# ssheybani/baby-vision-curriculum

Hardware: AMD Instinct MI355X
Metric: video clips/sec (node) VideoMAE-base 16x224^2 bf16 pretraining (higher is better)
Workload: dtype bf16; 1 GPU; VideoMAE-base (ViT-B/16 encoder, 4-layer decoder), 16x224x224 clips, tubelet 2, 90% tube mask, full training step (fwd + MSE + bwd + GradScaler + SGD-Nesterov); clips_per_gpu=256, global_batch=256, parallelism=dp1, weights=random init N(0,0.02), seed 0

## Files before the change

baby-vision-curriculum_amd/csrc/attention.hip:

```cpp
#include <stdlib.h>

#include "attention.h"

namespace bvc {

#define AS3 __attribute__((address_space(3)))
#define MFMA32(a, b, c) __builtin_amdgcn_mfma_f32_32x32x16_bf16((a), (b), (c), 0, 0, 0)

template <int HD>
__device__ __forceinline__ int swz_dual(int r) {
    if constexpr (HD == 64) return (((r >> 1) & 1) << 2) | ((r >> 2) & 3);
    else return (r >> 2) & 3;
}

template <int HD>
constexpr int pan_w(int p) { return HD - 64 * p >= 64 ? 64 : HD - 64 * p; }
constexpr int img_hd(int hd) { return hd == 80 || hd == 88 ? 96 : hd; }
constexpr uint32_t kDmaZero = 0xfffffff0u;
__device__ __forceinline__ int swz_pw(int pw, int r) { return pw == 64 ? swz_dual<64>(r) : swz_dual<32>(r); }

template <int PW, int NW, int VC = PW / 8>
__device__ __forceinline__ void stage_panel(__amdgpu_buffer_rsrc_t rs, int row0, int ld, int col0, char* lds, int GB, int wave, int lane) {
    constexpr int CPR = PW / 8;
    constexpr int RPP = 64 / CPR;
// ... 10 lines not shown
    }
}

template <int HD, int NW = 4, int HV = HD>
__device__ __forceinline__ void stage64(__amdgpu_buffer_rsrc_t rs, int row0, int ld, int col0, char* lds,
                                        int wave, int lane) {
    static_assert(HV == HD || (HD == 96 && HV > 64 && HV % 8 == 0), "stage64: a narrower head only on the 96 image");
    if constexpr (HD > 64) {
        stage_panel<64, NW>(rs, row0, ld, col0, lds, 16 * HD * 2, wave, lane);
        stage_panel<pan_w<HD>(1), NW, (HV - 64) / 8>(rs, row0, ld, col0 + 64, lds + 2048, 16 * HD * 2, wave, lane);
        return;
    }
    constexpr int CPR = HD / 8;
    constexpr int RPP = 64 / CPR;
#pragma unroll
    for (int jj = 0; jj < (HD / 8 + NW - 1) / NW; ++jj) {
        const int j = wave + NW * jj;
        if (NW > HD / 8 && j >= HD / 8) break;
        const int r = RPP * j + lane / CPR;
        const int c = (lane % CPR) ^ swz_dual<HD>(r);
        const uint32_t off = (uint32_t)(((size_t)(row0 + r) * ld + col0 + c * 8) * 2);
        glds16(rs, off, __builtin_amdgcn_readfirstlane((uint32_t)(size_t)((AS3 char*)lds) + (uint32_t)j * 1024u));
    }
}

template <int HD>
struct FragAddr {
    uint32_t rows[HD / 16];
    uint32_t tr[HD / 32][2];
};

template <int HD>
__device__ __forceinline__ FragAddr<HD> make_frag_addr(int lane) {
    FragAddr<HD> a;
    if constexpr (HD > 64) {
        constexpr int GB = 16 * HD * 2;
        const int r = lane & 31, h = lane >> 5, rg = r & 15;
#pragma unroll
        for (int st = 0; st < HD / 16; ++st) {
            const int pw = pan_w<HD>(st >> 2);
            a.rows[st] = (r >> 4) * GB + (st >> 2) * 2048 + rg * pw * 2 + (((2 * (st & 3) + h) ^ swz_pw(pw, rg)) << 4);
        }
        const int q = (lane >> 2) & 3, p = lane & 3;
#pragma unroll
        for (int t = 0; t < HD / 32; ++t) {
            const int pw = pan_w<HD>(t >> 1);
// ... 554 lines not shown
        bf16_t* krow = dqkv + (size_t)(b * N + ki) * ld + D + head * HD;
        bf16_t* vrow = krow + D;
#pragma unroll
        for (int t = 0; t < HI / 32; ++t)
#pragma unroll
            for (int g = 0; g < 4; ++g) {
                const int d = 32 * t + 8 * g + 4 * h;
                if (HD != HI && d >= HD) continue;
                uint2 a = {pack2bf(dk[t][4 * g] * scale, dk[t][4 * g + 1] * scale), pack2bf(dk[t][4 * g + 2] * scale, dk[t][4 * g + 3] * scale)};
                *reinterpret_cast<uint2*>(krow + d) = a;
                uint2 e = {pack2bf(dv[t][4 * g], dv[t][4 * g + 1]), pack2bf(dv[t][4 * g + 2], dv[t][4 * g + 3])};
                *reinterpret_cast<uint2*>(vrow + d) = e;
            }
    }
}

template <int HD, int NBT>
__global__ __launch_bounds__(320, 1) void attn_bwd_head_kernel(const bf16_t* __restrict__ qkv, const bf16_t* __restrict__ dctx,
                                                               const bf16_t* __restrict__ ctx, const float* __restrict__ lse,
                                                               bf16_t* __restrict__ dqkv, int N, int H, int D, int nheads,
                                                               uint32_t qkv_bytes, uint32_t dctx_bytes, float scale, float scale_log2) {
    static_assert(HD == 64, "whole-head backward: head_dim 64");
    extern __shared__ __attribute__((aligned(16))) char smem[];
    constexpr int IMG = 192 * HD * 2, SUB = 32 * HD * 2, KS = 16 * HD * 2;
    constexpr int QI = 0, KI = IMG, VI = 2 * IMG, OI = 3 * IMG;
    constexpr int STAT = 4 * IMG;
    constexpr int DST = STAT + 2 * 192 * 4;
    const AS3 char* lds = (const AS3 char*)smem;
    const int tid = threadIdx.x, lane = tid & 63;
    const int wave = __builtin_amdgcn_readfirstlane(tid >> 6);
    const int ld = 3 * D, h = lane >> 5;
    const int NB = NBT > 0 ? NBT : (N + 31) >> 5;
    const __amdgpu_buffer_rsrc_t rq = make_rsrc(qkv, qkv_bytes), rd = make_rsrc(dctx, dctx_bytes);
    const FragAddr<HD> fa = make_frag_addr<HD>(lane);
    const FragAddr<32> fs = make_frag_addr<32>(lane);

    auto stage_qvo = [&](int bh) __attribute__((always_inline)) {
        if (wave < 4) {
            const int b = bh / H, head = bh % H, row0 = b * N;
            for (int rb = 0; rb * 64 < N; ++rb) {
                stage64<HD>(rq, row0 + rb * 64, ld, head * HD, smem + QI + rb * 2 * SUB, wave, lane);
                stage64<HD>(rq, row0 + rb * 64, ld, 2 * D + head * HD, smem + VI + rb * 2 * SUB, wave, lane);
                stage64<HD>(rd, row0 + rb * 64, D, head * HD, smem + OI + rb * 2 * SUB, wave, lane);
            }
        }
    };
    auto stage_k = [&](int bh) __attribute__((always_inline)) {
        if (wave < 4) {
            const int b = bh / H, head = bh % H, row0 = b * N;
            for (int rb = 0; rb * 64 < N; ++rb) stage64<HD>(rq, row0 + rb * 64, ld, D + head * HD, smem + KI + rb * 2 * SUB, wave, lane);
        }
    };
    float st_lse = 0.f, st_del[5];
    auto load_stats = [&](int bh) __attribute__((always_inline)) {
        const int b = bh / H, head = bh % H;
        st_lse = (tid < N) ? lse[(size_t)bh * N + tid] : 0.f;
#pragma unroll
        for (int k = 0; k < 5; ++k) {
            const int q = (tid >> 3) + 40 * k, c = tid & 7;
            float acc = 0.f;
            if (q < N) {
                const bf16x8 dv = load8(dctx + (size_t)(b * N + q) * D + head * HD + 8 * c);
                const bf16x8 ov = load8(ctx + (size_t)(b * N + q) * D + head * HD + 8 * c);
#pragma unroll
                for (int j = 0; j < 8; ++j) acc += bf2f((bf16_t)dv[j]) * bf2f((bf16_t)ov[j]);
            }
            st_del[k] = acc;
        }
    };
    auto store_stats = [&]() __attribute__((always_inline)) {
        AS3 float* st = (AS3 float*)((AS3 char*)smem + STAT);
        if (tid < 192) st[tid] = st_lse;
#pragma unroll
        for (int k = 0; k < 5; ++k) {
            float acc = st_del[k];
            acc += __shfl_xor(acc, 1, 64);
            acc += __shfl_xor(acc, 2, 64);
            acc += __shfl_xor(acc, 4, 64);
            const int q = (tid >> 3) + 40 * k;
            if ((tid & 7) == 0 && q < 192) st[192 + q] = -acc;
        }
    };

    int bh = blockIdx.x;
    if (bh >= nheads) return;
    load_stats(bh);
    stage_qvo(bh);
    stage_k(bh);
    for (; bh < nheads; bh += gridDim.x) {
    const int b = bh / H, head = bh % H;
    const int nxt = bh + gridDim.x;
    asm volatile("s_waitcnt vmcnt(0)" ::: "memory");
    store_stats();
    __syncthreads();

    for (int kb = wave; kb < NB; kb += 5) {
        const int ki = kb * 32 + (lane & 31);
        bf16x8 kf[HD / 16], vf[HD / 16];
#pragma unroll
        for (int st = 0; st < HD / 16; ++st) {
            kf[st] = *reinterpret_cast<const AS3 bf16x8*>(lds + KI + kb * SUB + fa.rows[st]);
            vf[st] = *reinterpret_cast<const AS3 bf16x8*>(lds + VI + kb * SUB + fa.rows[st]);
        }
        f32x16 dk[HD / 32], dv[HD / 32];
#pragma unroll
        for (int t = 0; t < HD / 32; ++t) { dk[t] = zero16(); dv[t] = zero16(); }
        const bool key_ok = ki < N;
#pragma unroll
        for (int qb = 0; qb < (NBT > 0 ? NBT : NB); ++qb) {
            const AS3 char* qim = lds + QI + qb * SUB;
            const AS3 char* oim = lds + OI + qb * SUB;
            const AS3 float* stl = reinterpret_cast<const AS3 float*>(lds + STAT) + qb * 32 + 4 * h;
            f32x16 s = zero16(), dp;
#pragma unroll
            for (int g = 0; g < 4; ++g) {
                const f32x4 nd = *reinterpret_cast<const AS3 f32x4*>(stl + 192 + 8 * g);
#pragma unroll
                for (int e = 0; e < 4; ++e) dp[4 * g + e] = nd[e];
            }
#pragma unroll
            for (int stp = 0; stp < HD / 16; ++stp) {
                s = MFMA32(*reinterpret_cast<const AS3 bf16x8*>(qim + fa.rows[stp]), kf[stp], s);
                dp = MFMA32(*reinterpret_cast<const AS3 bf16x8*>(oim + fa.rows[stp]), vf[stp], dp);
            }
// ... 46 lines not shown
#pragma unroll
                for (int g = 0; g < 4; ++g) {
                    const int d = 32 * t + 8 * g + 4 * h;
                    uint2 a = {pack2bf(dk[t][4 * g] * scale, dk[t][4 * g + 1] * scale), pack2bf(dk[t][4 * g + 2] * scale, dk[t][4 * g + 3] * scale)};
                    *reinterpret_cast<uint2*>(krow + d) = a;
                    uint2 e = {pack2bf(dv[t][4 * g], dv[t][4 * g + 1]), pack2bf(dv[t][4 * g + 2], dv[t][4 * g + 3])};
                    *reinterpret_cast<uint2*>(vrow + d) = e;
                }
        }
    }
    __syncthreads();
    if (nxt < nheads) {
        stage_qvo(nxt);
        load_stats(nxt);
    }

    for (int qb = wave; qb < NB; qb += 5) {
        const int qi = qb * 32 + (lane & 31);
        f32x16 dq[HD / 32];
#pragma unroll
        for (int t = 0; t < HD / 32; ++t) dq[t] = zero16();
#pragma unroll
        for (int kb = 0; kb < (NBT > 0 ? NBT : NB); ++kb) {
            const AS3 char* kim = lds + KI + kb * SUB;
            const AS3 char* blk = lds + DST + (kb * 5 + qb) * 2048;
            const bf16x8 b0 = lds_tr<0>(blk, fs.tr[0][0], fs.tr[0][1]);
            const bf16x8 b1 = lds_tr<1024>(blk, fs.tr[0][0], fs.tr[0][1]);
#pragma unroll
            for (int t = 0; t < HD / 32; ++t) dq[t] = MFMA32(lds_tr<0>(kim, fa.tr[t][0], fa.tr[t][1]), b0, dq[t]);
#pragma unroll
            for (int t = 0; t < HD / 32; ++t) dq[t] = MFMA32(lds_tr<KS>(kim, fa.tr[t][0], fa.tr[t][1]), b1, dq[t]);
        }
        if (qi < N) {
            bf16_t* orow = dqkv + (size_t)(b * N + qi) * ld + head * HD;
#pragma unroll
            for (int t = 0; t < HD / 32; ++t)
#pragma unroll
                for (int g = 0; g < 4; ++g) {
                    const int d = 32 * t + 8 * g + 4 * h;
                    uint2 a = {pack2bf(dq[t][4 * g] * scale, dq[t][4 * g + 1] * scale), pack2bf(dq[t][4 * g + 2] * scale, dq[t][4 * g + 3] * scale)};
                    *reinterpret_cast<uint2*>(orow + d) = a;
                }
        }
    }
    __syncthreads();
    if (nxt < nheads) stage_k(nxt);
    }
}

static int xcd_remap() {
#ifdef BVC_EXPERIMENTS
    return getenv("BVC_ATTN_PLAIN_GRID") == nullptr;
#else
    return 1;
#endif
}

static bool head_kernel_enabled() {
#ifdef BVC_EXPERIMENTS
    return getenv("BVC_ATTN_NO_HEAD_KERNEL") == nullptr;
#else
    return true;
#endif
}

template <int HD>
static int fwd_hd(const bf16_t* qkv, bf16_t* ctx, float* lse, int B, int N, int H, hipStream_t stream, float sm_scale) {
    constexpr int HI = img_hd(HD);
    const int D = H * HD;
// ... 7 lines not shown
        BVC_CHECK_HIP(hipGetLastError());
        return BVC_OK;
    }
#endif
    const dim3 grid((unsigned)(((N + 127) / 128) * B * H));
    hipLaunchKernelGGL((attn_fwd_kernel<HD, 4>), grid, dim3(256), 4 * 64 * HI * 2, stream, qkv, ctx, lse, N, H, D, (uint32_t)bytes, scale_log2,
                       xcd_remap());
    BVC_CHECK_HIP(hipGetLastError());
    return BVC_OK;
}

template <int HD>
static int bwd_hd(const bf16_t* qkv, const bf16_t* ctx, const bf16_t* dctx, const float* lse, float* delta, bf16_t* dqkv, int B,
                  int N, int H, hipStream_t stream, float sm_scale, int parts) {
    constexpr int HI = img_hd(HD);
    const int D = H * HD;
    const size_t bytes = (size_t)B * N * 3 * D * 2;
    const float scale = sm_scale > 0.f ? sm_scale : 1.0f / sqrtf((float)HD), scale_log2 = scale * 1.4426950408889634f;
    const dim3 grid((unsigned)(((N + 127) / 128) * B * H));
    const int remap = xcd_remap();
    if constexpr (HD == 64) {
        if (parts == 3 && N <= 160 && head_kernel_enabled()) {
            constexpr size_t lds = 4 * 192 * HD * 2 + 2 * 192 * 4 + 25 * 2048;
            static bool attr_set = false;
            if (!attr_set) {
                BVC_CHECK_HIP(hipFuncSetAttribute(reinterpret_cast<const void*>(&attn_bwd_head_kernel<HD, 5>),
                                                  hipFuncAttributeMaxDynamicSharedMemorySize, (int)lds));
                BVC_CHECK_HIP(hipFuncSetAttribute(reinterpret_cast<const void*>(&attn_bwd_head_kernel<HD, 0>),
                                                  hipFuncAttributeMaxDynamicSharedMemorySize, (int)lds));
                attr_set = true;
            }
            static int ncu = 0;
            if (ncu == 0) {
                int dev = 0;
                hipDeviceProp_t prop;
                BVC_CHECK_HIP(hipGetDevice(&dev));
                BVC_CHECK_HIP(hipGetDeviceProperties(&prop, dev));
                ncu = prop.multiProcessorCount > 0 ? prop.multiProcessorCount : 256;
            }
            const int nheads = B * H;
            const dim3 g((unsigned)(nheads < ncu ? nheads : ncu));
            if (N > 128)
                hipLaunchKernelGGL((attn_bwd_head_kernel<HD, 5>), g, dim3(320), lds, stream, qkv, dctx, ctx, lse, dqkv, N, H, D, nheads,
                                   (uint32_t)bytes, (uint32_t)((size_t)B * N * D * 2), scale, scale_log2);
            else
                hipLaunchKernelGGL((attn_bwd_head_kernel<HD, 0>), g, dim3(320), lds, stream, qkv, dctx, ctx, lse, dqkv, N, H, D, nheads,
                                   (uint32_t)bytes, (uint32_t)((size_t)B * N * D * 2), scale, scale_log2);
            BVC_CHECK_HIP(hipGetLastError());
            return BVC_OK;
        }
    }
    if (parts & 1) {
#ifdef BVC_EXPERIMENTS
    if (HI == HD && getenv("BVC_ATTN_DQ_W") != nullptr) {
        constexpr int NB = 3;
        const dim3 gridw((unsigned)(((N + 32 * NB - 1) / (32 * NB)) * B * H));
        hipLaunchKernelGGL((attn_bwd_dq_w_kernel<HI, NB>), gridw, dim3(64), kRing * 2 * 32 * HI * 2, stream, qkv, dctx, ctx, lse, delta, dqkv, N, H, D,
                           (uint32_t)bytes, scale, scale_log2, remap);
    } else
#endif
    hipLaunchKernelGGL(attn_bwd_dq_kernel<HD>, grid, dim3(256), 4 * 64 * HI * 2, stream, qkv, dctx, ctx, lse, delta, dqkv, N, H, D,
                       (uint32_t)bytes, scale, scale_log2, remap);
    }
    if (parts & 2) {
    constexpr int lds_dkdv = 2 * (2 * 64 * HI * 2 + 512);
    if constexpr (lds_dkdv > 65536) {
// ... 51 lines not shown
```

baby-vision-curriculum_amd/csrc/rowops.h:

```cpp
#pragma once
#include "common.h"
#include "dropgate.h"

namespace bvc {

struct RowMap { int rin, rout, roff; };
static inline RowMap identity_rows() { return RowMap{0, 0, 0}; }

struct PatchGeom { int T, C, H, W, ts, ps; };

struct PixelSrc {
    const void* ptr;
    int is_u8;
    float mean[4], stdv[4];
};
static inline PixelSrc pixels_f32(const float* p) { return PixelSrc{p, 0, {0, 0, 0, 0}, {1, 1, 1, 1}}; }

int launch_ln_fwd(const float* x, RowMap rm, const float* gamma, const float* beta, bf16_t* y, float* mean, float* rstd,
                  int M, int D, float eps, hipStream_t s, float* y32 = nullptr);
size_t ln_bwd_workspace_floats(int M, int D);
size_t ln_bwd_workspace_floats_upto(int Mmax, int D);
int launch_ln_bwd(const bf16_t* dy, const float* x, RowMap rm, const float* mean, const float* rstd, const float* gamma,
                  float* dres, int accumulate, bf16_t* dres_bf, float* dgamma, float* dbeta, float* part, int M, int D, hipStream_t s,
                  const Gate* gate = nullptr);
int launch_ln_param_reduce(const float* part, int nblk, int D, float* dgamma, float* dbeta, hipStream_t s);
int launch_colsum_bf16(const bf16_t* X, int M, int N, int ld, float alpha, float* out, hipStream_t s);
int launch_colsum_bf16_scaled(const bf16_t* X, int M, int N, int ld, float alpha, const float* alpha_dev, float* out, hipStream_t s);
int launch_colsum_f32(const float* X, RowMap rm, int M, int D, float* out, hipStream_t s);
int launch_token_mean(const float* x, int B, int N, int D, float* out, hipStream_t s);
int launch_token_mean_bwd(const float* dmean, int B, int N, int D, float* dx, hipStream_t s);
int launch_fcnorm_bwd_bcast(const float* dy, const float* p, const float* mean, const float* rstd, const float* gamma, float* dres,
                            bf16_t* dres_bf, float* dgamma, float* dbeta, int B, int N, int D, hipStream_t s, const Gate* gate = nullptr);
int launch_dropout_mask(const Gate& gate, size_t n, uint8_t* out, hipStream_t s);
void dropout_mask_host(const Gate& gate, size_t n, uint8_t* out);
int launch_cast_bf16(const float* in, bf16_t* out, size_t n, hipStream_t s);
int launch_gather_rows_bf16(const float* in, RowMap rm, bf16_t* out, int M, int D, hipStream_t s);
int launch_mask_index(const uint8_t* mask, int B, int L, int nvis, int nmask, int* vis_idx, int* msk_idx, int* status, hipStream_t s);
int launch_dual_mask_index(const uint8_t* mask, const uint8_t* decode, int B, int L, int nvis, int ndec, int* vis_idx, int* dec_idx,
                           int* status, hipStream_t s);
int launch_gather_patches(PixelSrc clip, const int* vis_idx, bf16_t* A, int B, int nvis, PatchGeom pg, hipStream_t s);
int launch_labels(PixelSrc clip, const int* dec_idx, float* labels, int B, int ndec, PatchGeom pg, int norm_pix, hipStream_t s);
int launch_fill_masked(float* xfull, const float* mask_token, const float* pos, const int* dec_idx, int B, int Ld, int nvis,
                       int ndec, int D, hipStream_t s);
int launch_sgd_step(float* p, float* g, float* buf, size_t n, float lr, float momentum, float dampening, float wd, int nesterov,
                    int first, int maximize, const float* grad_scale, const float* found_inf, int write_grad, bf16_t* shadow,
                    hipStream_t s);
int launch_adam_prep(float* state, double lr, double beta1, double beta2, const float* found_inf, hipStream_t s);
int launch_adam_step(float* p, float* g, float* m, float* v, size_t n, double lr, double beta1, double beta2, double eps, double wd,
                     int decoupled, int maximize, const float* state, const float* grad_scale, const float* found_inf, int write_grad,
                     bf16_t* shadow, hipStream_t s);
int launch_sgd_step_segments(float* p, float* g, float* buf, int64_t n, const int64_t* seg_start, const int* seg_group, const int* blk_seg,
                             int nseg, const bvc_sgd_groups* groups, const float* grad_scale, const float* found_inf, int write_grad,
                             bf16_t* shadow, hipStream_t s);
int launch_adam_step_segments(float* p, float* g, float* m, float* v, int64_t n, const int64_t* seg_start, const int* seg_group,
                              const int* blk_seg, int nseg, const bvc_adam_groups* groups, float* state, double* hyper_dev,
                              const float* grad_scale, const float* found_inf, int write_grad, bf16_t* shadow, hipStream_t s);
int launch_pad_heads(const bf16_t* wqkv, const float* bqkv, const bf16_t* wo, bf16_t* wqkv_p, float* bqkv_p, bf16_t* wo_p, int D, int H,
                     int hd, int hdp, hipStream_t s);
int launch_unpad_head_grads(const float* gwqkv_p, const float* gbqkv_p, const float* gwo_p, float* gwqkv, float* gbqkv, float* gwo, int D,
// ... 18 lines not shown
```

baby-vision-curriculum_amd/csrc/rowops.hip:

```cpp
#include "rowops.h"
#include "gemm.h"

#include <algorithm>

namespace bvc {

constexpr int kMaxChunks = 4;
constexpr int kWideChunks = 6;

__device__ __forceinline__ int map_row(int m, RowMap rm) {
    return rm.rin > 0 ? (m / rm.rin) * rm.rout + rm.roff + (m % rm.rin) : m;
}

template <int LPR>
__device__ __forceinline__ float row_sum(float v) {
#pragma unroll
    for (int o = LPR / 2; o > 0; o >>= 1) v += __shfl_xor(v, o, 64);
    return v;
}

template <int LPR, int NC>
__global__ __launch_bounds__(256) void ln_fwd_kernel(const float* __restrict__ x, RowMap rm, const float* __restrict__ gamma,
                                                     const float* __restrict__ beta, bf16_t* __restrict__ y, float* __restrict__ y32,
                                                     float* __restrict__ mean, float* __restrict__ rstd, int M, int D, float eps) {
// ... 405 lines not shown
#pragma unroll
    for (int e = 0; e < 4; ++e)
        if (q * 4 + e < n) out[q * 4 + e] = r[e] >= gate.thr ? 1 : 0;
}

__global__ void cast_f32_bf16_kernel(const float* __restrict__ in, bf16_t* __restrict__ out, size_t n) {
    const size_t i = ((size_t)blockIdx.x * blockDim.x + threadIdx.x) * 8;
    if (i + 8 <= n) {
        const f32x4 a = *reinterpret_cast<const f32x4*>(in + i);
        const f32x4 b = *reinterpret_cast<const f32x4*>(in + i + 4);
        *reinterpret_cast<uint4*>(out + i) = uint4{pack2bf(a[0], a[1]), pack2bf(a[2], a[3]), pack2bf(b[0], b[1]), pack2bf(b[2], b[3])};
    } else {
        for (size_t j = i; j < n; ++j) out[j] = f2bf(in[j]);
    }
}

__global__ void gather_rows_bf16_kernel(const float* __restrict__ in, RowMap rm, bf16_t* __restrict__ out, int M, int D) {
    const size_t i = (size_t)blockIdx.x * blockDim.x + threadIdx.x;
    const int nch = D >> 2;
    if (i >= (size_t)M * nch) return;
    const int m = (int)(i / nch), c = (int)(i % nch);
    const f32x4 v = *reinterpret_cast<const f32x4*>(in + (size_t)map_row(m, rm) * D + c * 4);
    *reinterpret_cast<uint2*>(out + (size_t)m * D + c * 4) = uint2{pack2bf(v[0], v[1]), pack2bf(v[2], v[3])};
}

__global__ void mask_index_kernel(const uint8_t* __restrict__ mask, int L, int nvis, int nmask, int* __restrict__ vis_idx,
                                  int* __restrict__ msk_idx, int* __restrict__ status) {
    const int b = blockIdx.x, lane = threadIdx.x;
    int nv = 0, nm = 0;
    const unsigned long long below = lane == 0 ? 0ull : (~0ull >> (64 - lane));
    for (int base = 0; base < L; base += 64) {
        const int t = base + lane;
        const bool in = t < L;
        const bool mk = in && mask[(size_t)b * L + t] != 0;
        const unsigned long long bm = __ballot(mk), bv = __ballot(in && !mk);
        if (mk) { const int p = nm + __popcll(bm & below); if (p < nmask) msk_idx[(size_t)b * nmask + p] = t; }
        if (in && !mk) { const int p = nv + __popcll(bv & below); if (p < nvis) vis_idx[(size_t)b * nvis + p] = t; }
        nm += __popcll(bm);
        nv += __popcll(bv);
    }
    if (lane == 0 && (nv != nvis || nm != nmask)) atomicOr(status, 1);
}

__global__ void dual_mask_index_kernel(const uint8_t* __restrict__ mask, const uint8_t* __restrict__ decode, int L, int nvis, int ndec,
                                       int* __restrict__ vis_idx, int* __restrict__ dec_idx, int* __restrict__ status) {
    const int b = blockIdx.x, lane = threadIdx.x;
// ... 884 lines not shown
            hipLaunchKernelGGL(fcnorm_bwd_bcast_gate_kernel, dim3(std::max(chunks, pcols), B + 1), dim3(256), 0, s, dy, p, mean, rstd, gamma, dres,
                               dres_bf, dgamma, dbeta, B, N, D, B, *gate);
        } else {
            hipLaunchKernelGGL(fcnorm_bwd_bcast_kernel, dim3(std::max(chunks, pcols), B + 1), dim3(256), 0, s, dy, p, mean, rstd, gamma, dres,
                               dres_bf, dgamma, dbeta, B, N, D, B);
        }
    }
    BVC_CHECK_HIP(hipGetLastError());
    return BVC_OK;
}

int launch_cast_bf16(const float* in, bf16_t* out, size_t n, hipStream_t s) {
    hipLaunchKernelGGL(cast_f32_bf16_kernel, dim3(blocks_for((n + 7) / 8)), dim3(256), 0, s, in, out, n);
    BVC_CHECK_HIP(hipGetLastError());
    return BVC_OK;
}

int launch_gather_rows_bf16(const float* in, RowMap rm, bf16_t* out, int M, int D, hipStream_t s) {
    hipLaunchKernelGGL(gather_rows_bf16_kernel, dim3(blocks_for((size_t)M * (D / 4))), dim3(256), 0, s, in, rm, out, M, D);
    BVC_CHECK_HIP(hipGetLastError());
    return BVC_OK;
}

int launch_mask_index(const uint8_t* mask, int B, int L, int nvis, int nmask, int* vis_idx, int* msk_idx, int* status, hipStream_t s) {
    hipLaunchKernelGGL(mask_index_kernel, dim3(B), dim3(64), 0, s, mask, L, nvis, nmask, vis_idx, msk_idx, status);
    BVC_CHECK_HIP(hipGetLastError());
    return BVC_OK;
}

int launch_dual_mask_index(const uint8_t* mask, const uint8_t* decode, int B, int L, int nvis, int ndec, int* vis_idx, int* dec_idx,
                           int* status, hipStream_t s) {
    hipLaunchKernelGGL(dual_mask_index_kernel, dim3(B), dim3(64), 0, s, mask, decode, L, nvis, ndec, vis_idx, dec_idx, status);
    BVC_CHECK_HIP(hipGetLastError());
    return BVC_OK;
}

int launch_gather_patches(PixelSrc clip, const int* vis_idx, bf16_t* A, int B, int nvis, PatchGeom pg, hipStream_t s) {
    BVC_REQUIRE(pg.ps % 8 == 0 && pg.W % 4 == 0, "gather_patches: patch size must be a multiple of 8");
    const size_t items = (size_t)B * nvis * (pg.C * pg.ts * pg.ps * pg.ps / 8);
    hipLaunchKernelGGL(gather_patches_kernel, dim3(blocks_for(items)), dim3(256), 0, s, clip, vis_idx, A, B, nvis, pg);
    BVC_CHECK_HIP(hipGetLastError());
    return BVC_OK;
}

int launch_labels(PixelSrc clip, const int* dec_idx, float* labels, int B, int ndec, PatchGeom pg, int norm_pix, hipStream_t s) {
    BVC_REQUIRE(pg.ps % 4 == 0, "labels: patch size must be a multiple of 4");
// ... 227 lines not shown
```

baby-vision-curriculum_amd/csrc/videomae.hip:

```cpp
#include <math.h>
#include <stdarg.h>
#include <stdio.h>
#include <stdlib.h>
#include <string.h>

#include <algorithm>
#include <string>
#include <vector>

#include "stack.h"

namespace bvc {
static thread_local char g_err[1024] = "";
void set_error(const char* fmt, ...) {
    va_list ap;
    va_start(ap, fmt);
    vsnprintf(g_err, sizeof(g_err), fmt, ap);
    va_end(ap);
}
const char* last_error() { return g_err; }
}

using namespace bvc;

// ... 306 lines not shown
    }
    const RowMap tail{ndec, Ld, nvis};
    TRY(launch_ln_fwd(c->dec.x_out, tail, params + L.norm_w, params + L.norm_b, c->lnf, c->meanf, c->rstdf, Mm, Dd, cf.decoder_norm_eps, st));
    TRY(launch_labels(pixels, c->dec_idx, c->labels, B, ndec, pg, cf.norm_pix_loss, st));
    {
        GemmProblem p = gemm(c->lnf, (size_t)Mm * Dd, Dd, c->wbf + L.head_w, (size_t)P * Dd, Dd, Mm, P, Dd, EPI_LOSS, c->diff, P);
        p.bias = params + L.head_b; p.labels = c->labels; p.partial = c->partial; p.C2 = logits;
        c->npartial = gemm_num_tiles(p, -1);
        TRY(launch_gemm(&p, 1, GEMM_NT, -1, st));
    }
    TRY(launch_loss_finalize(c->partial, c->npartial, (double)Mm * (double)P, c->status, loss, st));
    c->have_forward = true;
    return BVC_OK;
}

int bvc_videomae_backward(bvc_ctx* c, const float* grad_loss, float* G, bvc_bucket_fn on_bucket, void* user, void* stream) {
    BVC_REQUIRE(c && grad_loss && G, "backward: null argument");
    if (!c->have_forward) { set_error("backward: no forward state (call bvc_videomae_forward first; one backward per forward)"); return BVC_ERR_STATE; }
    c->have_forward = false;
    hipStream_t st = (hipStream_t)stream;
    const bvc_videomae_config& cf = c->cfg;
    const Layout& L = c->lay;
    const int B = c->batch, nvis = c->nvis, ndec = c->ndec, Ld = c->Ld;
    const int Mv = B * nvis, Md = B * Ld, Mm = B * ndec;
    const int D = cf.hidden_size, Dd = cf.decoder_hidden_size, P = c->P;
    const bf16_t* W = c->wbf;
    const float* params = c->params;
    auto bucket = [&](int64_t lo, int64_t hi) { if (on_bucket) on_bucket(lo, hi - lo, user); };
    begin_backward(c->w);

    BVC_CHECK_HIP(hipMemsetAsync(G, 0, (size_t)L.total * 4, st));
    const float cmse = (float)(2.0 / ((double)Mm * (double)P));
    {
        GemmProblem p = gemm(c->diff, (size_t)Mm * P, P, c->lnf, (size_t)Mm * Dd, Dd, P, Dd, Mm, EPI_F32, G + L.head_w, Dd);
        p.alpha = cmse; p.alpha_dev = grad_loss;
        p.rowsum = G + L.head_b;
        const int tile = plan_dw(&p, 1);
        TRY(launch_gemm(&p, 1, GEMM_TN, tile, st));
    }
    {
        GemmProblem p = gemm(c->diff, (size_t)Mm * P, P, W + L.head_w, (size_t)P * Dd, Dd, Mm, Dd, P, EPI_BF16, c->w.dln, Dd);
        p.alpha = cmse; p.alpha_dev = grad_loss;
        TRY(launch_gemm(&p, 1, GEMM_NN, -1, st));
    }
    BVC_CHECK_HIP(hipMemsetAsync(c->dres_dec, 0, (size_t)Md * Dd * 4, st));
    BVC_CHECK_HIP(hipMemsetAsync(c->w.dyb[0], 0, (size_t)Md * Dd * 2, st));
    const RowMap tail{ndec, Ld, nvis};
    TRY(launch_ln_bwd(c->w.dln, c->dec.x_out, tail, c->meanf, c->rstdf, params + L.norm_w, c->dres_dec, 0, c->w.dyb[0],
                      G + L.norm_w, G + L.norm_b, c->w.ln_part, Mm, Dd, st));
    bucket(L.norm_w, L.total);
    for (int i = c->dec.nlayers - 1; i >= 0; --i) {
        TRY(layer_backward(c->w, c->dec, i, L.dec[i], c->dec.act[i].x_in, c->dres_dec, G, B, Ld, st, on_bucket, user));
    }
    TRY(launch_colsum_f32(c->dres_dec, tail, Mm, Dd, G + L.mask_token, st));
    const RowMap headrows{nvis, Ld, 0};
    TRY(launch_gather_rows_bf16(c->dres_dec, headrows, c->de2d, Mv, Dd, st));
    {
        GemmProblem p = gemm(c->de2d, (size_t)Mv * Dd, Dd, c->xe_bf, (size_t)Mv * D, D, Dd, D, Mv, EPI_F32, G + L.e2d_w, D);
        const int tile = plan_dw(&p, 1);
        TRY(launch_gemm(&p, 1, GEMM_TN, tile, st));
    }
    {
        GemmProblem p = gemm(c->de2d, (size_t)Mv * Dd, Dd, W + L.e2d_w, (size_t)Dd * D, D, Mv, D, Dd, EPI_F32_BF16, c->dres_enc, D);
        p.C2 = c->w.dyb[c->w.seq % 3];
        TRY(launch_gemm(&p, 1, GEMM_NN, -1, st));
    }
    bucket(L.e2d_w, L.dec.front().ln1w);
    for (int i = c->enc.nlayers - 1; i >= 0; --i) {
        TRY(layer_backward(c->w, c->enc, i, L.enc[i], c->enc.act[i].x_in, c->dres_enc, G, B, nvis, st, on_bucket, user));
    }
    {
        GemmProblem p = gemm(c->w.dyb[c->w.seq % 3], (size_t)Mv * D, D, c->Ape, (size_t)Mv * c->Kp, c->Kp, D, c->Kp, Mv, EPI_F32, G + L.pe_w, c->Kp);
        p.rowsum = G + L.pe_b;
        const int tile = plan_dw(&p, 1);
        TRY(launch_gemm(&p, 1, GEMM_TN, tile, st));
    }
    TRY(join_side(c->w, c->w.seq & 1, st, on_bucket, user));
    TRY(join_side(c->w, (c->w.seq + 1) & 1, st, on_bucket, user));
// ... 554 lines not shown
```

baby-vision-curriculum_amd/jepa.py:

```python
from __future__ import annotations

import ctypes
import math
from functools import partial

import numpy as np
import torch
import torch.nn as nn

from . import _lib
from .dropgate import BranchGate
from .flat import FlatParamModule, query_layout


def apply_masks(x, masks):
    all_x = []
    for m in masks:
        mask_keep = m.unsqueeze(-1).repeat(1, 1, x.size(-1))
        all_x += [torch.gather(x, dim=1, index=mask_keep)]
    return torch.cat(all_x, dim=0)


def repeat_interleave_batch(x, B, repeat):
    N = len(x) // B
# ... 109 lines not shown

    @property
    def num_patches(self):
        return self._pe_info.num_patches

    @property
    def drop_path_scale(self):
        return self._gate.scale

    def _get_ctx(self, batch):
        dev = self._flat.device.index
        if self._ctx is not None and self._ctx_key[1] == dev and self._ctx_key[0] >= batch:
            return self._ctx
        self._free_ctx()
        h = ctypes.c_void_p()
        _lib.check(_lib.lib().bvc_vit_create(ctypes.byref(self._cfg), batch, ctypes.byref(h)), "bvc_vit_create")
        self._ctx, self._ctx_key = h, (batch, dev)
        return h

    def _free_ctx(self):
        if getattr(self, "_ctx", None) is not None:
            _lib.lib().bvc_vit_destroy(self._ctx)
            self._ctx = None

    def __del__(self):
        try:
            self._free_ctx()
        except Exception:
            pass

    def _run_forward(self, imgs, idx):
        B = imgs.shape[0]
        N = idx.shape[1] if idx is not None else self.num_patches
        h = self._get_ctx(B)
        out = torch.empty((B, N, self.embed_dim), dtype=torch.float32, device=imgs.device)
        fmt = _lib.pixel_format(imgs, self.pixel_mean, self.pixel_std, self.in_chans)
        self._shadow_vouch(h)
        if self.training and self._gate.enabled:
            self._gate.arm(_lib.lib().bvc_vit_set_drop, h, imgs.device, B, N)
        _lib.check(_lib.lib().bvc_vit_forward_px(h, imgs.data_ptr(), ctypes.byref(fmt) if fmt is not None else None,
                                                 idx.data_ptr() if idx is not None else None, B, N, self._flat.data_ptr(),
                                                 out.data_ptr(), _lib.current_stream_ptr()), "bvc_vit_forward")
        self._shadow_established(h)
        self._live = (imgs, idx)
        return out

# ... 80 lines not shown
        self._init_flat(layout, numel, init, frozen=("predictor_pos_embed",))
        self._ctx, self._ctx_key = None, None

    @property
    def drop_path_scale(self):
        return self._gate.scale

    def _get_ctx(self, B, nsets, tokens):
        dev = self._flat.device.index
        k = self._ctx_key
        if self._ctx is not None and k[3] == dev and k[0] >= B and k[1] >= nsets and k[2] >= tokens:
            return self._ctx
        self._free_ctx()
        h = ctypes.c_void_p()
        tokens = max(tokens, min(2 * self.num_patches, tokens + 64))
        _lib.check(_lib.lib().bvc_predictor_create(ctypes.byref(self._cfg), B, nsets, tokens, ctypes.byref(h)), "bvc_predictor_create")
        self._ctx, self._ctx_key = h, (B, nsets, tokens, dev)
        return h

    def _free_ctx(self):
        if getattr(self, "_ctx", None) is not None:
            _lib.lib().bvc_predictor_destroy(self._ctx)
            self._ctx = None

    def __del__(self):
        try:
            self._free_ctx()
        except Exception:
            pass

    def _run_forward(self, z, idx_ctx, idx_pred):
        B, Nc = idx_ctx.shape
        nsets, _, Np = idx_pred.shape
        h = self._get_ctx(B, nsets, Nc + Np)
        zf = z.detach().to(torch.float32).contiguous()
        out = torch.empty((nsets * B, Np, self.embed_dim), dtype=torch.float32, device=z.device)
        self._shadow_vouch(h)
        if self.training and self._gate.enabled:
            self._gate.arm(_lib.lib().bvc_predictor_set_drop, h, z.device, nsets * B, Nc + Np)
        _lib.check(_lib.lib().bvc_predictor_forward(h, zf.data_ptr(), idx_ctx.data_ptr(), idx_pred.data_ptr(), B, Nc, nsets, Np,
                                                    self._flat.data_ptr(), out.data_ptr(), _lib.current_stream_ptr()),
                   "bvc_predictor_forward")
        self._shadow_established(h)
        self._live = (zf, idx_ctx, idx_pred)
        return out

# ... 207 lines not shown
```

baby-vision-curriculum_amd/videomae.py:

```python
from __future__ import annotations

import ctypes
import warnings
from dataclasses import dataclass
from typing import Optional

import torch
import torch.nn as nn

from . import _lib
from .dropgate import BranchGate
from .flat import FlatParamModule, query_layout


class VideoMAEConfig:

    def __init__(self, image_size=224, patch_size=16, num_channels=3, num_frames=16, tubelet_size=2,
                 hidden_size=768, num_hidden_layers=12, num_attention_heads=12, intermediate_size=3072,
                 hidden_act="gelu", layer_norm_eps=1e-12, initializer_range=0.02, qkv_bias=True,
                 use_mean_pooling=True, decoder_num_attention_heads=6, decoder_hidden_size=384,
                 decoder_num_hidden_layers=4, decoder_intermediate_size=1536, norm_pix_loss=True,
                 hidden_dropout_prob=0.0, attention_probs_dropout_prob=0.0, drop_path_rate=0.0,
                 output_hidden_states=False, output_attentions=False, **kwargs):
        self.output_hidden_states, self.output_attentions = bool(output_hidden_states), bool(output_attentions)
# ... 139 lines not shown
            "bool_decode_pos: the number of decoded patches per clip changed (or differs between clips, or a decoded patch was not "
            "masked) without a new model object; every clip must decode the same number of its masked patches",
            "every clip must have the same number of decoded patches")
        self.pixel_mean, self.pixel_std = 0.5, 0.25

    def _get_ctx(self, batch, nmask, ndec=None):
        key = (batch, nmask, self._flat.device.index, nmask if ndec is None else ndec)
        if self._ctx is not None and self._ctx_key[1:] == key[1:] and self._ctx_key[0] >= batch:
            return self._ctx
        self._free_ctx()
        h = ctypes.c_void_p()
        cc = self.config.to_c()
        if ndec is None:
            _lib.check(_lib.lib().bvc_videomae_create(ctypes.byref(cc), batch, nmask, ctypes.byref(h)), "bvc_videomae_create")
        else:
            _lib.check(_lib.lib().bvc_videomae_create_dual(ctypes.byref(cc), batch, nmask, ndec, ctypes.byref(h)), "bvc_videomae_create_dual")
        self._ctx, self._ctx_key = h, key
        return h

    def _free_ctx(self):
        if self._ctx is not None:
            _lib.lib().bvc_videomae_destroy(self._ctx)
            self._ctx = None

    def __del__(self):
        try:
            self._free_ctx()
        except Exception:
            pass

    def _num_masked(self, mask):
        return self._mask_count.count(mask, self.strict_mask_check)

    def _num_decoded(self, decode, mask):
        return self._decode_count.count(decode, self.strict_mask_check, bad=(decode & ~mask).any(),
                                        bad_message="bool_decode_pos must be a subset of bool_masked_pos: a decoded patch is visible to the encoder")

    def _run_forward(self, pixels, mask, decode, want_logits):
        cfg = self.config
        fmt = _lib.pixel_format(pixels, self.pixel_mean, self.pixel_std, cfg.num_channels)
        B = pixels.shape[0]
        nmask = self._num_masked(mask)
        ndec = self._num_decoded(decode, mask) if decode is not None else None
        h = self._get_ctx(B, nmask, ndec)
        loss = torch.empty((), dtype=torch.float32, device=pixels.device)
        logits = None
# ... 238 lines not shown
        self._ctx = None
        self._ctx_key = None
        self._train = _TrainCtx()
        self._warned_eval_grad = False
        self.pixel_mean, self.pixel_std = 0.5, 0.25

    def _get_ctx(self, batch):
        key = (batch, self._flat.device.index)
        if self._ctx is not None and self._ctx_key[1] == key[1] and self._ctx_key[0] >= batch:
            return self._ctx
        self._free_ctx()
        h = ctypes.c_void_p()
        cc = self.config.to_c()
        _lib.check(_lib.lib().bvc_videomae_encoder_create(ctypes.byref(cc), batch, ctypes.byref(h)), "bvc_videomae_encoder_create")
        self._ctx, self._ctx_key = h, key
        return h

    def _get_train_ctx(self, batch):
        t = self._train
        key = (batch, self._flat.device.index)
        if t.h is not None and t.key[1] == key[1] and t.key[0] >= batch:
            return t.h
        t.free()
        h = ctypes.c_void_p()
        cc = self.config.to_c()
        _lib.check(_lib.lib().bvc_videomae_cls_create(ctypes.byref(cc), batch, ctypes.byref(h)), "bvc_videomae_cls_create")
        t.h, t.key = h, key
        return h

    def _shadow_ctx(self):
        return self._train.h

    def __deepcopy__(self, memo):
        import copy
        new = super().__deepcopy__(memo)
        new.fc_norm = copy.deepcopy(self.fc_norm, memo)
        new.classifier = copy.deepcopy(self.classifier, memo)
        return new

    def _free_ctx(self):
        if self._ctx is not None:
            _lib.lib().bvc_videomae_encoder_destroy(self._ctx)
            self._ctx = None

    def __del__(self):
        try:
# ... 149 lines not shown
```

Measured before the change: 3281 clips/s.

## Double-buffer K in whole-head attention backward and zero only head rows in decoder grad

For the N=160 whole-head attention backward, the K image is double-buffered in LDS with exact 160-row staging. The next head's K is prefetched right after the stats barrier instead of after a trailing __syncthreads, which removes that barrier and overlaps the load with compute. Separately, the full memsets of the decoder residual gradient buffers are replaced by a kernel that zeroes only the visible head rows, because the tail rows are overwritten by layer-norm backward. The Python destroy paths also invalidate shadow state. The extra LDS image raises LDS use per block, and the narrower zeroing depends on the tail rows really being overwritten.

Result: no change. 3282 clips/s (median of 3 runs) (+0.0%).

```diff
diff --git a/baby-vision-curriculum_amd/csrc/attention.hip b/baby-vision-curriculum_amd/csrc/attention.hip
--- a/baby-vision-curriculum_amd/csrc/attention.hip
+++ b/baby-vision-curriculum_amd/csrc/attention.hip
@@ -56,6 +56,13 @@
         const uint32_t off = (uint32_t)(((size_t)(row0 + r) * ld + col0 + c * 8) * 2);
         glds16(rs, off, __builtin_amdgcn_readfirstlane((uint32_t)(size_t)((AS3 char*)lds) + (uint32_t)j * 1024u));
     }
+}
+
+__device__ __forceinline__ void stage32(__amdgpu_buffer_rsrc_t rs, int row0, int ld, int col0, char* lds, int wave, int lane) {
+    const int r = 8 * wave + lane / 8;
+    const int c = (lane % 8) ^ swz_dual<64>(r);
+    const uint32_t off = (uint32_t)(((size_t)(row0 + r) * ld + col0 + c * 8) * 2);
+    glds16(rs, off, __builtin_amdgcn_readfirstlane((uint32_t)(size_t)((AS3 char*)lds) + (uint32_t)wave * 1024u));
 }
 
 template <int HD>
@@ -656,9 +663,12 @@
                                                                uint32_t qkv_bytes, uint32_t dctx_bytes, float scale, float scale_log2) {
     static_assert(HD == 64, "whole-head backward: head_dim 64");
     extern __shared__ __attribute__((aligned(16))) char smem[];
-    constexpr int IMG = 192 * HD * 2, SUB = 32 * HD * 2, KS = 16 * HD * 2;
+    constexpr bool K2 = NBT == 5;
+    constexpr int ROWS = K2 ? 160 : 192;
+    constexpr int IMG = ROWS * HD * 2, SUB = 32 * HD * 2, KS = 16 * HD * 2;
     constexpr int QI = 0, KI = IMG, VI = 2 * IMG, OI = 3 * IMG;
-    constexpr int STAT = 4 * IMG;
+    constexpr int KJ = 4 * IMG;
+    constexpr int STAT = (K2 ? 5 : 4) * IMG;
     constexpr int DST = STAT + 2 * 192 * 4;
     const AS3 char* lds = (const AS3 char*)smem;
     const int tid = threadIdx.x, lane = tid & 63;
@@ -669,20 +679,35 @@
     const FragAddr<HD> fa = make_frag_addr<HD>(lane);
     const FragAddr<32> fs = make_frag_addr<32>(lane);
 
+    auto stage_img = [&](__amdgpu_buffer_rsrc_t rs, int row0, int ldi, int col0, char* img) __attribute__((always_inline)) {
+        if constexpr (K2) {
+            stage64<HD>(rs, row0, ldi, col0, img, wave, lane);
+            stage64<HD>(rs, row0 + 64, ldi, col0, img + 2 * SUB, wave, lane);
+            stage32(rs, row0 + 128, ldi, col0, img + 4 * SUB, wave, lane);
+        } else {
+            for (int rb = 0; rb * 64 < N; ++rb) stage64<HD>(rs, row0 + rb * 64, ldi, col0, img + rb * 2 * SUB, wave, lane);
+        }
+    };
     auto stage_qvo = [&](int bh) __attribute__((always_inline)) {
         if (wave < 4) {
             const int b = bh / H, head = bh % H, row0 = b * N;
-            for (int rb = 0; rb * 64 < N; ++rb) {
-                stage64<HD>(rq, row0 + rb * 64, ld, head * HD, smem + QI + rb * 2 * SUB, wave, lane);
-                stage64<HD>(rq, row0 + rb * 64, ld, 2 * D + head * HD, smem + VI + rb * 2 * SUB, wave, lane);
-                stage64<HD>(rd, row0 + rb * 64, D, head * HD, smem + OI + rb * 2 * SUB, wave, lane);
+            if constexpr (K2) {
+                stage_img(rq, row0, ld, head * HD, smem + QI);
+                stage_img(rq, row0, ld, 2 * D + head * HD, smem + VI);
+                stage_img(rd, row0, D, head * HD, smem + OI);
+            } else {
+                for (int rb = 0; rb * 64 < N; ++rb) {
+                    stage64<HD>(rq, row0 + rb * 64, ld, head * HD, smem + QI + rb * 2 * SUB, wave, lane);
+                    stage64<HD>(rq, row0 + rb * 64, ld, 2 * D + head * HD, smem + VI + rb * 2 * SUB, wave, lane);
+                    stage64<HD>(rd, row0 + rb * 64, D, head * HD, smem + OI + rb * 2 * SUB, wave, lane);
+                }
             }
         }
     };
-    auto stage_k = [&](int bh) __attribute__((always_inline)) {
+    auto stage_k = [&](int bh, int kofs) __attribute__((always_inline)) {
         if (wave < 4) {
             const int b = bh / H, head = bh % H, row0 = b * N;
-            for (int rb = 0; rb * 64 < N; ++rb) stage64<HD>(rq, row0 + rb * 64, ld, D + head * HD, smem + KI + rb * 2 * SUB, wave, lane);
+            stage_img(rq, row0, ld, D + head * HD, smem + kofs);
         }
     };
     float st_lse = 0.f, st_del[5];
@@ -720,20 +745,24 @@
     if (bh >= nheads) return;
     load_stats(bh);
     stage_qvo(bh);
-    stage_k(bh);
+    stage_k(bh, KI);
+    int kofs = KI;
     for (; bh < nheads; bh += gridDim.x) {
     const int b = bh / H, head = bh % H;
     const int nxt = bh + gridDim.x;
     asm volatile("s_waitcnt vmcnt(0)" ::: "memory");
     store_stats();
     __syncthreads();
+    if constexpr (K2) {
+        if (nxt < nheads) stage_k(nxt, kofs ^ (KI ^ KJ));
+    }
 
     for (int kb = wave; kb < NB; kb += 5) {
         const int ki = kb * 32 + (lane & 31);
         bf16x8 kf[HD / 16], vf[HD / 16];
 #pragma unroll
         for (int st = 0; st < HD / 16; ++st) {
-            kf[st] = *reinterpret_cast<const AS3 bf16x8*>(lds + KI + kb * SUB + fa.rows[st]);
+            kf[st] = *reinterpret_cast<const AS3 bf16x8*>(lds + kofs + kb * SUB + fa.rows[st]);
             vf[st] = *reinterpret_cast<const AS3 bf16x8*>(lds + VI + kb * SUB + fa.rows[st]);
         }
         f32x16 dk[HD / 32], dv[HD / 32];
@@ -826,7 +855,7 @@
         for (int t = 0; t < HD / 32; ++t) dq[t] = zero16();
 #pragma unroll
         for (int kb = 0; kb < (NBT > 0 ? NBT : NB); ++kb) {
-            const AS3 char* kim = lds + KI + kb * SUB;
+            const AS3 char* kim = lds + kofs + kb * SUB;
             const AS3 char* blk = lds + DST + (kb * 5 + qb) * 2048;
             const bf16x8 b0 = lds_tr<0>(blk, fs.tr[0][0], fs.tr[0][1]);
             const bf16x8 b1 = lds_tr<1024>(blk, fs.tr[0][0], fs.tr[0][1]);
@@ -847,8 +876,12 @@
                 }
         }
     }
-    __syncthreads();
-    if (nxt < nheads) stage_k(nxt);
+    if constexpr (K2) {
+        kofs ^= KI ^ KJ;
+    } else {
+        __syncthreads();
+        if (nxt < nheads) stage_k(nxt, KI);
+    }
     }
 }
 
@@ -902,10 +935,12 @@
     if constexpr (HD == 64) {
         if (parts == 3 && N <= 160 && head_kernel_enabled()) {
             constexpr size_t lds = 4 * 192 * HD * 2 + 2 * 192 * 4 + 25 * 2048;
+            constexpr size_t lds5 = 5 * 160 * HD * 2 + 2 * 192 * 4 + 25 * 2048;
+            static_assert(lds5 <= 160 * 1024, "whole-head backward: LDS of a CU");
             static bool attr_set = false;
             if (!attr_set) {
                 BVC_CHECK_HIP(hipFuncSetAttribute(reinterpret_cast<const void*>(&attn_bwd_head_kernel<HD, 5>),
-                                                  hipFuncAttributeMaxDynamicSharedMemorySize, (int)lds));
+                                                  hipFuncAttributeMaxDynamicSharedMemorySize, (int)lds5));
                 BVC_CHECK_HIP(hipFuncSetAttribute(reinterpret_cast<const void*>(&attn_bwd_head_kernel<HD, 0>),
                                                   hipFuncAttributeMaxDynamicSharedMemorySize, (int)lds));
                 attr_set = true;
@@ -921,7 +956,7 @@
             const int nheads = B * H;
             const dim3 g((unsigned)(nheads < ncu ? nheads : ncu));
             if (N > 128)
-                hipLaunchKernelGGL((attn_bwd_head_kernel<HD, 5>), g, dim3(320), lds, stream, qkv, dctx, ctx, lse, dqkv, N, H, D, nheads,
+                hipLaunchKernelGGL((attn_bwd_head_kernel<HD, 5>), g, dim3(320), lds5, stream, qkv, dctx, ctx, lse, dqkv, N, H, D, nheads,
                                    (uint32_t)bytes, (uint32_t)((size_t)B * N * D * 2), scale, scale_log2);
             else
                 hipLaunchKernelGGL((attn_bwd_head_kernel<HD, 0>), g, dim3(320), lds, stream, qkv, dctx, ctx, lse, dqkv, N, H, D, nheads,
diff --git a/baby-vision-curriculum_amd/csrc/rowops.h b/baby-vision-curriculum_amd/csrc/rowops.h
--- a/baby-vision-curriculum_amd/csrc/rowops.h
+++ b/baby-vision-curriculum_amd/csrc/rowops.h
@@ -35,6 +35,7 @@
 void dropout_mask_host(const Gate& gate, size_t n, uint8_t* out);
 int launch_cast_bf16(const float* in, bf16_t* out, size_t n, hipStream_t s);
 int launch_gather_rows_bf16(const float* in, RowMap rm, bf16_t* out, int M, int D, hipStream_t s);
+int launch_zero_rows(float* x, bf16_t* xb, RowMap rm, int M, int D, hipStream_t s);
 int launch_mask_index(const uint8_t* mask, int B, int L, int nvis, int nmask, int* vis_idx, int* msk_idx, int* status, hipStream_t s);
 int launch_dual_mask_index(const uint8_t* mask, const uint8_t* decode, int B, int L, int nvis, int ndec, int* vis_idx, int* dec_idx,
                            int* status, hipStream_t s);
diff --git a/baby-vision-curriculum_amd/csrc/rowops.hip b/baby-vision-curriculum_amd/csrc/rowops.hip
--- a/baby-vision-curriculum_amd/csrc/rowops.hip
+++ b/baby-vision-curriculum_amd/csrc/rowops.hip
@@ -451,6 +451,16 @@
     const int m = (int)(i / nch), c = (int)(i % nch);
     const f32x4 v = *reinterpret_cast<const f32x4*>(in + (size_t)map_row(m, rm) * D + c * 4);
     *reinterpret_cast<uint2*>(out + (size_t)m * D + c * 4) = uint2{pack2bf(v[0], v[1]), pack2bf(v[2], v[3])};
+}
+
+__global__ void zero_rows_kernel(float* __restrict__ x, bf16_t* __restrict__ xb, RowMap rm, int M, int D) {
+    const size_t i = (size_t)blockIdx.x * blockDim.x + threadIdx.x;
+    const int nch = D >> 2;
+    if (i >= (size_t)M * nch) return;
+    const int m = (int)(i / nch), c = (int)(i % nch);
+    const size_t at = (size_t)map_row(m, rm) * D + c * 4;
+    *reinterpret_cast<f32x4*>(x + at) = f32x4{0, 0, 0, 0};
+    *reinterpret_cast<uint2*>(xb + at) = uint2{0u, 0u};
 }
 
 __global__ void mask_index_kernel(const uint8_t* __restrict__ mask, int L, int nvis, int nmask, int* __restrict__ vis_idx,
@@ -1381,6 +1391,14 @@
     return BVC_OK;
 }
 
+int launch_zero_rows(float* x, bf16_t* xb, RowMap rm, int M, int D, hipStream_t s) {
+    BVC_REQUIRE(D % 4 == 0, "zero_rows: D = %d is not a multiple of 4", D);
+    if (M <= 0) return BVC_OK;
+    hipLaunchKernelGGL(zero_rows_kernel, dim3(blocks_for((size_t)M * (D / 4))), dim3(256), 0, s, x, xb, rm, M, D);
+    BVC_CHECK_HIP(hipGetLastError());
+    return BVC_OK;
+}
+
 int launch_mask_index(const uint8_t* mask, int B, int L, int nvis, int nmask, int* vis_idx, int* msk_idx, int* status, hipStream_t s) {
     hipLaunchKernelGGL(mask_index_kernel, dim3(B), dim3(64), 0, s, mask, L, nvis, nmask, vis_idx, msk_idx, status);
     BVC_CHECK_HIP(hipGetLastError());
diff --git a/baby-vision-curriculum_amd/csrc/videomae.hip b/baby-vision-curriculum_amd/csrc/videomae.hip
--- a/baby-vision-curriculum_amd/csrc/videomae.hip
+++ b/baby-vision-curriculum_amd/csrc/videomae.hip
@@ -352,7 +352,7 @@
     const bvc_videomae_config& cf = c->cfg;
     const Layout& L = c->lay;
     const int B = c->batch, nvis = c->nvis, ndec = c->ndec, Ld = c->Ld;
-    const int Mv = B * nvis, Md = B * Ld, Mm = B * ndec;
+    const int Mv = B * nvis, Mm = B * ndec;
     const int D = cf.hidden_size, Dd = cf.decoder_hidden_size, P = c->P;
     const bf16_t* W = c->wbf;
     const float* params = c->params;
@@ -373,8 +373,8 @@
         p.alpha = cmse; p.alpha_dev = grad_loss;
         TRY(launch_gemm(&p, 1, GEMM_NN, -1, st));
     }
-    BVC_CHECK_HIP(hipMemsetAsync(c->dres_dec, 0, (size_t)Md * Dd * 4, st));
-    BVC_CHECK_HIP(hipMemsetAsync(c->w.dyb[0], 0, (size_t)Md * Dd * 2, st));
+    const RowMap headrows{nvis, Ld, 0};
+    TRY(launch_zero_rows(c->dres_dec, c->w.dyb[0], headrows, Mv, Dd, st));
     const RowMap tail{ndec, Ld, nvis};
     TRY(launch_ln_bwd(c->w.dln, c->dec.x_out, tail, c->meanf, c->rstdf, params + L.norm_w, c->dres_dec, 0, c->w.dyb[0],
                       G + L.norm_w, G + L.norm_b, c->w.ln_part, Mm, Dd, st));
@@ -383,7 +383,6 @@
         TRY(layer_backward(c->w, c->dec, i, L.dec[i], c->dec.act[i].x_in, c->dres_dec, G, B, Ld, st, on_bucket, user));
     }
     TRY(launch_colsum_f32(c->dres_dec, tail, Mm, Dd, G + L.mask_token, st));
-    const RowMap headrows{nvis, Ld, 0};
     TRY(launch_gather_rows_bf16(c->dres_dec, headrows, c->de2d, Mv, Dd, st));
     {
         GemmProblem p = gemm(c->de2d, (size_t)Mv * Dd, Dd, c->xe_bf, (size_t)Mv * D, D, Dd, D, Mv, EPI_F32, G + L.e2d_w, D);
diff --git a/baby-vision-curriculum_amd/jepa.py b/baby-vision-curriculum_amd/jepa.py
--- a/baby-vision-curriculum_amd/jepa.py
+++ b/baby-vision-curriculum_amd/jepa.py
@@ -155,6 +155,7 @@
         if getattr(self, "_ctx", None) is not None:
             _lib.lib().bvc_vit_destroy(self._ctx)
             self._ctx = None
+            self._shadow_invalidate()
 
     def __del__(self):
         try:
@@ -281,6 +282,7 @@
         if getattr(self, "_ctx", None) is not None:
             _lib.lib().bvc_predictor_destroy(self._ctx)
             self._ctx = None
+            self._shadow_invalidate()
 
     def __del__(self):
         try:
diff --git a/baby-vision-curriculum_amd/videomae.py b/baby-vision-curriculum_amd/videomae.py
--- a/baby-vision-curriculum_amd/videomae.py
+++ b/baby-vision-curriculum_amd/videomae.py
@@ -185,6 +185,7 @@
         if self._ctx is not None:
             _lib.lib().bvc_videomae_destroy(self._ctx)
             self._ctx = None
+            self._shadow_invalidate()
 
     def __del__(self):
         try:
@@ -469,6 +470,7 @@
         if t.h is not None and t.key[1] == key[1] and t.key[0] >= batch:
             return t.h
         t.free()
+        self._shadow_invalidate()
         h = ctypes.c_void_p()
         cc = self.config.to_c()
         _lib.check(_lib.lib().bvc_videomae_cls_create(ctypes.byref(cc), batch, ctypes.byref(h)), "bvc_videomae_cls_create")
```
